# paulffm/Continuous-Time-Diffusion-Models-for-Discrete-Data

Hardware: AMD Instinct MI355X
Metric: tau-leaping sample-steps/s (higher is better)
Workload: dtype bf16; 1 GPU; MNIST tauLDR U-Net TauL step (config_tauUnet_mnist: D=784, S=256, 1000-step grid); batch_per_gpu=256, global_batch=256, D=784, S=256, parallelism=sample-sharded x1, no collective in the loop

## Files before the change

### continuous-time-diffusion-models-for-discrete-data_amd/ctdd/native.py

```python
import ctypes as C
import os

import torch

_HERE = os.path.dirname(os.path.dirname(os.path.abspath(__file__)))
_LIB = None

BRANCH_CTELBO, BRANCH_CRM = 0, 1
LOGIT_TYPES = {"direct": 0, "reverse_prob": 1, "reverse_logscale": 2}
STEP_ORDINAL, STEP_CORRECTOR, STEP_COUNT_RAW, STEP_CRM, STEP_COUNT_JUMPS, STEP_BF16, STEP_LOGITS_BF16 = 1, 2, 4, 8, 16, 32, 64


class CtddError(RuntimeError):
    pass


def lib_path():
    return os.environ.get("CTDD_LIBRARY") or os.path.join(_HERE, "libctdd.so")


_P, _I, _F, _U64, _U32, _I64 = C.c_void_p, C.c_int, C.c_float, C.c_uint64, C.c_uint32, C.c_int64
_SIGS = {
    "ctdd_abi_version": ([], _I),
    "ctdd_last_error": ([], C.c_char_p),
    "ctdd_rate_table": ([_P, _P, _P, _P, _P, _P, _I, _I, _I, _F, _P, _P, _P, _P, _P], _I),
    "ctdd_noise_categorical": ([_P, _P, _P, _P, _U64, _U64, _I, _I, _I, _P, _P], _I),
    "ctdd_xtilde_sample": ([_P, _P, _P, _P, _P, _U64, _U64, _I, _I, _I, _P, _P, _P, _P], _I),
    "ctdd_xtilde_sample_masked": ([_P, _P, _P, _P, _P, _P, _U64, _U64, _I, _I, _I, _P, _P, _P, _P], _I),
    "ctdd_logprob": ([_P, _P, _P, _P, _I, _I, _I, _I, _P, _P, _P], _I),
    "ctdd_reverse_rates": ([_I, _I, _P, _P, _P, _P, _P, _F, _I, _I, _I, _P, _P, _P], _I),
    "ctdd_tauleap_apply": ([_P, _P, _P, _I, _I, _I, _I, _P, _P, _P], _I),
    "ctdd_tauleap_draw": ([_P, _P, _P, _F, _U32, _U64, _U64, _I, _I, _I, _P, _P, _P], _I),
    "ctdd_tauleap_step": ([_I, _I, _P, _P, _P, _P, _P, _F, _F, _F, _U32, _U64, _U64, _I, _I, _I, _P, _P, _P], _I),
    "ctdd_tauleap_step_rows": ([_I, _I, _P, _P, _P, _P, _P, _F, _F, _F, _U32, _U64, _U64, _I, _I, _I, _P, _I, _P, _P, _P], _I),
    "ctdd_lbjf_step": ([_I, _I, _P, _P, _P, _P, _F, _F, _F, _U32, _P, _U64, _U64, _I, _I, _I, _P, _P, _P, _P], _I),
    "ctdd_logprob_rp_mfma": ([_P, _P, _P, _I, _I, _I, _P, _P, _P, _P], _I),
    "ctdd_logprob_rp_bwd_mfma": ([_P, _P, _P, _P, _P, _F, _I, _I, _I, _P, _P, _P, _P, _P], _I),
    "ctdd_exact_step": ([_P, _P, _P, _P, _P, _U64, _U64, _I, _I, _I, _P, _P, _P, _P], _I),
    "ctdd_midpoint_predict": ([_I, _I, _P, _P, _P, _P, _F, _F, _F, _I, _I, _I, _P, _P], _I),
    "ctdd_lbjf_from_rates": ([_P, _P, _F, _P, _U64, _U64, _I, _I, _I, _P, _P, _P, _P], _I),
    "ctdd_midpoint_from_rates": ([_P, _P, _F, _I, _I, _I, _P, _P], _I),
    "ctdd_lbjf_step_rows": ([_I, _I, _P, _P, _P, _P, _F, _F, _F, _U32, _P, _U64, _U64, _I, _I, _I, _P, _I, _P, _P, _P, _P], _I),
    "ctdd_midpoint_predict_rows": ([_I, _I, _P, _P, _P, _P, _F, _F, _F, _I, _I, _I, _P, _I, _P, _P], _I),
    "ctdd_exact_step_rows": ([_P, _P, _P, _P, _P, _U64, _U64, _I, _I, _I, _P, _I, _P, _P, _P, _P], _I),
    "ctdd_lbjf_from_rates_rows": ([_P, _P, _F, _P, _U64, _U64, _I, _I, _I, _P, _I, _P, _P, _P, _P], _I),
    "ctdd_midpoint_from_rates_rows": ([_P, _P, _F, _I, _I, _I, _P, _I, _P, _P], _I),
    "ctdd_argmax": ([_P, _I, _I, _I, _P, _P], _I),
    "ctdd_initial_samples": ([_P, _U64, _U64, _I, _I, _I, _P, _P], _I),
    "ctdd_philox_uniform": ([_U64, _U64, _I64, _I, _P, _P], _I),
    "ctdd_s256_step_table_bytes": ([], _I64),
    "ctdd_s256_prepare": ([_P, _P, _F, _I, _P, _P, _P, _P], _I),
    "ctdd_s256_prepare_crm": ([_P, _P, _I, _P, _P, _P, _P], _I),
    "ctdd_tauleap_step_s256": ([_P, _P, _P, _P, _P, _P, _F, _F, _U32, _U64, _U64, _I, _I, _P, _P, _P, _P], _I),
    "ctdd_tauleap_step_s256_rows": ([_P, _P, _P, _P, _P, _P, _F, _F, _U32, _U64, _U64, _I, _I, _P, _I, _P, _P, _P, _P], _I),
    "ctdd_crm_loss": ([_P, _P, _P, _P, _I, _I, _I, _I, _F, _F, _P, _P, _P, _P], _I),
    "ctdd_ctelbo_scratch_bytes": ([_I, _I, _I], _I64),
    "ctdd_ctelbo_loss": ([_P, _P, _P, _P, _P, _P, _I, _I, _I, _F, _F, _F, _P, _P, _P, _P], _I),
    "ctdd_ctelbo_loss_terms": ([_P, _P, _P, _P, _P, _P, _I, _I, _I, _F, _F, _F, _F, _P, _P, _P, _P], _I),
    "ctdd_ctelbo_loss_window": ([_P, _P, _P, _P, _P, _P, _I, _I, _I, _I, _I, _F, _F, _F, _F, _P, _P, _P, _P], _I),
    "ctdd_ctelbo_loss_masked": ([_P, _P, _P, _P, _P, _P, _P, _I, _I, _I, _F, _F, _F, _F, _P, _P, _P, _P], _I),
    "ctdd_score_elbo_loss": ([_P, _P, _P, _P, _P, _P, _I, _I, _I, _F, _F, _P, _P, _P, _P], _I),
    "ctdd_crm_loss_ll": ([_P, _P, _P, _I, _I, _I, _I, _F, _P, _P, _P, _P], _I),
    "ctdd_score_elbo_loss_ll": ([_P, _P, _P, _P, _P, _P, _I, _I, _I, _F, _F, _P, _P, _P, _P], _I),
    "ctdd_logprob_bwd": ([_I, _P, _P, _P, _P, _P, _F, _I, _I, _I, _P, _P, _P, _P], _I),
    "ctdd_crm_loss_masked": ([_P, _P, _P, _P, _P, _I, _I, _I, _I, _F, _F, _P, _P, _P, _P], _I),
    "ctdd_crm_loss_ll_masked": ([_P, _P, _P, _P, _I, _I, _I, _I, _F, _P, _P, _P, _P], _I),
    "ctdd_score_elbo_loss_masked": ([_P, _P, _P, _P, _P, _P, _P, _I, _I, _I, _F, _F, _P, _P, _P, _P], _I),
    "ctdd_score_elbo_loss_ll_masked": ([_P, _P, _P, _P, _P, _P, _P, _I, _I, _I, _F, _F, _P, _P, _P, _P], _I),
    "ctdd_opt_chunk_elems": ([], _I),
    "ctdd_adam_ema_step": ([_P, _P, _I, _F, _F, _F, _F, _I64, _F, _F, _P, _P], _I),
    "ctdd_grad_sumsq": ([_P, _P, _I, _P, _I, _P], _I),
    "ctdd_adam_ema_apply": ([_P, _P, _I, _F, _F, _F, _F, _I64, _F, _F, _P, _P], _I),
}
UNET_EXPORTS = ("ctdd_unet_conv", "ctdd_unet_conv_patch", "ctdd_unet_conv_res", "ctdd_unet_conv_ring", "ctdd_unet_conv_up_phases", "ctdd_unet_upsample2x", "ctdd_unet_first_conv", "ctdd_unet_gn_apply", "ctdd_unet_gn_onepass", "ctdd_unet_channel_stats",
                "ctdd_unet_time", "ctdd_unet_time_uniform", "ctdd_unet_attention", "ctdd_unet_logistic_head", "ctdd_unet_resblock_small",
                "ctdd_unet_resblock_mid", "ctdd_unet_conv_rows", "ctdd_unet_conv_rows_head")
HOLLOW_EXPORTS = ("ctdd_gemm_bf16", "ctdd_hollow_small_linear", "ctdd_hollow_embed", "ctdd_hollow_layernorm", "ctdd_hollow_add", "ctdd_hollow_put_rows", "ctdd_hollow_attention", "ctdd_hollow_attention_bf16")
UNET_TRAIN_EXPORTS = ("ctdd_unet_wgrad", "ctdd_unet_gn_bwd", "ctdd_unet_dropout", "ctdd_unet_colsum", "ctdd_unet_sum_batch", "ctdd_unet_sum_jobs", "ctdd_unet_accumulate",
                      "ctdd_unet_downsum2x", "ctdd_unet_upsample2x_f32", "ctdd_unet_cast_rows", "ctdd_unet_attention_bwd",
                      "ctdd_unet_first_conv_wgrad", "ctdd_unet_first_conv_wgrad_scratch", "ctdd_unet_pack_weights",
                      "ctdd_unet_unpack_grads")
HOLLOW_TRAIN_EXPORTS = ("ctdd_hollow_layernorm_bwd", "ctdd_hollow_attention_train", "ctdd_hollow_attention_bwd", "ctdd_hollow_attention_train_bf16", "ctdd_hollow_attention_bwd_bf16", "ctdd_hollow_act", "ctdd_hollow_relu_bf16", "ctdd_hollow_colsum", "ctdd_hollow_dropout",
                        "ctdd_hollow_embed_bwd")
BERT_EXPORTS = ("ctdd_bert_embed", "ctdd_bert_gather", "ctdd_bert_attention_short",
                "ctdd_bert_embed_bwd", "ctdd_bert_gather_bwd",
                "ctdd_bert_embed_enum_bwd", "ctdd_bert_gather_enum_bwd",
                "ctdd_bert_attention_short_train", "ctdd_bert_attention_short_bwd")
EXPORTS = tuple(_SIGS) + UNET_EXPORTS + HOLLOW_EXPORTS + UNET_TRAIN_EXPORTS + HOLLOW_TRAIN_EXPORTS + BERT_EXPORTS


def load():
    global _LIB
    if _LIB is None:
        path = lib_path()
        if not os.path.exists(path):
            raise CtddError(f"{path} not found: build it with `python __graft_entry__.py` "
                            "(hipcc --offload-arch=gfx950); there is no CPU fallback")
        lib = C.CDLL(path)
        for name, (argt, rest) in _SIGS.items():
            fn = getattr(lib, name)
            fn.argtypes, fn.restype = argt, rest
        _LIB = lib
    return _LIB


def _ptr(t, dtype=None, name="tensor"):
    if t is None:
        return None
    if not isinstance(t, torch.Tensor):
        raise CtddError(f"{name}: expected a torch tensor, got {type(t)}")
    if not t.is_cuda:
        raise CtddError(f"{name}: must live on a GPU (got {t.device}); libctdd has no CPU path")
    if dtype is not None and t.dtype != dtype:
        raise CtddError(f"{name}: expected {dtype}, got {t.dtype}")
    if not t.is_contiguous():
        raise CtddError(f"{name}: must be contiguous")
    return t.data_ptr()


def _stream():
    return torch.cuda.current_stream().cuda_stream


def _check(rc, what):
    if rc != 0:
        msg = load().ctdd_last_error().decode(errors="replace")
        raise CtddError(f"{what} failed with status {rc}: {msg}")


f32, i32 = torch.float32, torch.int32


def rate_table(eigvecs, right, eigvals, base_rate, integral, beta, S, normalise, clamp_below=1e-8,
               want_qt0=True, want_qt0T=False, want_rate=False, want_noise_probs=False):
    nT = integral.numel()
    dev = integral.device
    mk = lambda want: torch.empty((nT, S, S), dtype=f32, device=dev) if want else None
    q, qT, r, pn = mk(want_qt0), mk(want_qt0T), mk(want_rate), mk(want_noise_probs)
    rc = load().ctdd_rate_table(_ptr(eigvecs, f32, "eigvecs"), _ptr(right, f32, "right"), _ptr(eigvals, f32, "eigvals"),
                                _ptr(base_rate, f32, "base_rate"), _ptr(integral, f32, "integral"),
                                _ptr(beta, f32, "beta"), nT, S, int(bool(normalise)), float(clamp_below),
                                _ptr(q), _ptr(qT), _ptr(r), _ptr(pn), _stream())
    _check(rc, "ctdd_rate_table")
    return q, qT, r, pn


def noise_categorical(probs, x0, tidx=None, E=None, seed=0, offset=0):
    B, D = x0.shape
    S = probs.shape[-1]
    out = torch.empty((B, D), dtype=i32, device=x0.device)
    rc = load().ctdd_noise_categorical(_ptr(probs, f32, "probs"), _ptr(tidx, i32, "tidx"), _ptr(x0, i32, "x0"),
                                       _ptr(E, f32, "E"), seed, offset, B, D, S, _ptr(out), _stream())
    _check(rc, "ctdd_noise_categorical")
    return out


def xtilde_sample(rate, x_t, tidx=None, E_dim=None, E_val=None, seed=0, offset=0):
    B, D = x_t.shape
    S = rate.shape[-1]
# ... 577 lines not shown
```

### continuous-time-diffusion-models-for-discrete-data_amd/ctdd/unet_engine.py

```python
import contextlib
import ctypes as C

import torch

from . import native
from .plan_launch import bound_launch, graph_capture, ptr

_P, _I, _F = C.c_void_p, C.c_int, C.c_float
SEG_3x3, SEG_1x1, SEG_3x3_S2, SEG_3x3_UP = 0, 1, 2, 3


class _Seg(C.Structure):
    _fields_ = [("hi", _P), ("f32", _P), ("C", _I), ("kind", _I)]


class _ConvArgs(C.Structure):
    _fields_ = [("seg", _Seg * 3), ("nseg", _I), ("w_hi", _P), ("w_f32", _P), ("B", _I), ("H", _I), ("W", _I),
                ("Hin", _I), ("Win", _I), ("N", _I), ("Ktot", _I), ("bias", _P), ("tbias", _P), ("tb_stride", _I),
                ("res_f32", _P), ("res_bf16", _P), ("out_f32", _P), ("out_hi", _P), ("stats", _P), ("logits_C", _I),
                ("ksplit", _I), ("acc_buf", _P), ("act", _I), ("out_lo", _P)]


class _FirstArgs(C.Structure):
    _fields_ = [("x64", _P), ("x32", _P), ("lo", _F), ("hi", _F), ("w", _P), ("bias", _P), ("B", _I), ("Cin", _I),
                ("H", _I), ("W", _I), ("Cout", _I), ("out_f32", _P), ("out_hi", _P), ("stats", _P), ("x0_f32", _P)]


class _GnArgs(C.Structure):
    _fields_ = [("s1_f32", _P), ("s1_bf16", _P), ("st1", _P), ("C1", _I), ("s2_f32", _P), ("s2_bf16", _P), ("st2", _P),
                ("C2", _I), ("gamma", _P), ("beta", _P), ("B", _I), ("HW", _I), ("G", _I), ("eps", _F), ("swish", _I),
                ("out_hi", _P), ("out_f32", _P)]


class _ResblockArgs(C.Structure):
    _fields_ = [("s1_bf16", _P), ("s2_bf16", _P), ("C1", _I), ("C2", _I), ("gamma1", _P), ("beta1", _P), ("gamma2", _P), ("beta2", _P),
                ("G1", _I), ("G2", _I), ("eps1", _F), ("eps2", _F), ("w1", _P), ("bias1", _P), ("tbias", _P), ("tb_stride", _I),
                ("w2", _P), ("bias2", _P), ("skip", _I), ("B", _I), ("H", _I), ("W", _I), ("N", _I), ("out_bf16", _P)]


class _ConvRowsArgs(C.Structure):
    _fields_ = [("s1_bf16", _P), ("st1", _P), ("C1", _I), ("s2_bf16", _P), ("st2", _P), ("C2", _I), ("gamma", _P), ("beta", _P), ("G", _I),
                ("eps", _F), ("w", _P), ("bias", _P), ("tbias", _P), ("tb_stride", _I), ("r1_bf16", _P), ("RC1", _I), ("r2_bf16", _P),
                ("RC2", _I), ("res_bf16", _P), ("out_bf16", _P), ("out_stats", _P), ("B", _I), ("H", _I), ("W", _I), ("N", _I)]


class _TimeArgs(C.Structure):
    _fields_ = [("t", _P), ("B", _I), ("ch", _I), ("tdim", _I), ("w1", _P), ("b1", _P), ("w2", _P), ("b2", _P),
                ("hid", _P), ("act", _P)]


class _AttnArgs(C.Structure):
    _fields_ = [("qkv", _P), ("B", _I), ("T", _I), ("C", _I), ("heads", _I), ("out_hi", _P), ("out_f32", _P)]


class _LogisticArgs(C.Structure):
    _fields_ = [("net", _P), ("x0", _P), ("B", _I), ("C", _I), ("HW", _I), ("S", _I), ("fix", _I), ("out", _P), ("fast", _I), ("out_bf16", _P)]


_sigs_done = False


def _lib():
    global _sigs_done
    lib = native.load()
    if not _sigs_done:
        for name, argt in (("ctdd_unet_conv", [_P, _I, _I, _I, _P]), ("ctdd_unet_conv_patch", [_P, _I, _I, _I, _P]), ("ctdd_unet_conv_res", [_P, _I, _P]), ("ctdd_unet_conv_ring", [_P, _I, _P]),
                           ("ctdd_unet_conv_up_phases", [_P, _I, _P]), ("ctdd_unet_upsample2x", [_P, _I, _I, _I, _I, _P, _P]), ("ctdd_unet_first_conv", [_P, _P]),
                           ("ctdd_unet_gn_apply", [_P, _P]), ("ctdd_unet_gn_onepass", [_P, _I, _I, _P]), ("ctdd_unet_channel_stats", [_P, _I, _I, _I, _P, _P]),
                           ("ctdd_unet_time", [_P, _P, _P, _I, _P, _P]), ("ctdd_unet_time_uniform", [_P, _P, _P, _I, _P, _P]),
                           ("ctdd_unet_attention", [_P, _P]), ("ctdd_unet_resblock_small", [_P, _I, _P]),
                           ("ctdd_unet_resblock_mid", [_P, _I, _P]), ("ctdd_unet_conv_rows", [_P, _I, _P]),
                           ("ctdd_unet_conv_rows_head", [_P, _I, _P]),
                           ("ctdd_unet_logistic_head", [_P, _P])):
            fn = getattr(lib, name)
            fn.argtypes, fn.restype = argt, _I
        _sigs_done = True
    return lib


def _unwrap(net):
    return net.module if hasattr(net, "module") and net.__class__.__name__ == "DistributedDataParallel" else net


def supports(model):
    net = _unwrap(getattr(model, "net", None))
    return (net is not None and net.__class__.__name__ == "UNet" and not model.padding
            and model.cfg.model.model_output in ("logits", "logistic_pars"))


def training_supported(model):
    if getattr(model.cfg.model, "engine_train", "hip") != "hip" or not supports(model):
        return False
    net = _unwrap(model.net)
    return net.channel % 16 == 0 and all((net.channel * int(m_)) % 16 == 0 for m_ in model.cfg.model.ch_mult)



def resblock_small_covers(H, W, cs, cout, G1, G2):
    Ct = sum(cs)
    if H * W > 64 or W > 8 or cout != 192 or len(cs) > 2 or any(c % 64 for c in cs) or Ct > 384 or Ct % G1 or cout % G2:
        return False
    if H * W > 16 and (H - 1) * (W + 2) + W > 80:
        return False
    rs_a, rs_2, prows = Ct * 2 + 32, cout * 2 + 32, (H + 2) * (W + 2)
    return H * W * rs_a + prows * max(rs_a, rs_2) + 256 * 80 + 2 * 384 * 8 + 2 * 384 * 4 <= 160 * 1024


def pack_resblock_weights(w2d):
    N, K = w2d.shape
    assert N == 192 and K % 64 == 0
    return w2d.reshape(4, 3, 16, K // 64, 2, 4, 8).permute(0, 3, 1, 4, 5, 2, 6).contiguous().reshape(N, K)


def resblock_mid_covers(H, W, cs, cout, G1, G2):
    Ct = sum(cs)
    if (H < 1 or W < 1 or H > 14 or W > 14 or cout != 192 or not 1 <= len(cs) <= 2
            or any(c <= 0 or c % 32 or c > 192 for c in cs) or G1 <= 0 or G2 <= 0 or Ct % G1 or cout % G2):
        return False
    return ((H + 2) * 16 + 2) * (cout * 2 + 32) + 256 * 80 + 2 * 384 * 8 + 2 * 384 * 4 <= 160 * 1024


def pack_row_tile_weights(w, cs, rcs, streams):
    N, Ct, Rt = w.shape[0], sum(cs), sum(rcs)
    assert N == 48 * streams and w.shape[1] == 9 * Ct + Rt and all(c % 32 == 0 for c in [*cs, *rcs])
    w3, parts, c0 = w[:, :9 * Ct].reshape(N, 9, Ct), [], 0
    for c in cs:
        v = w3[:, :, c0:c0 + c].reshape(streams, 3, 16, 3, 3, c // 32, 4, 8)
        parts.append(v.permute(0, 5, 4, 3, 1, 6, 2, 7).reshape(streams, -1))
        c0 += c
    c0 = 9 * Ct
    for c in rcs:
        v = w[:, c0:c0 + c].reshape(streams, 3, 16, c // 32, 4, 8)
        parts.append(v.permute(0, 3, 1, 4, 2, 5).reshape(streams, -1))
        c0 += c
    return torch.cat(parts, 1).contiguous().reshape(N, w.shape[1])


def pack_resblock_mid_weights(w1, w2, cs):
    N = w1.shape[0]
    return pack_row_tile_weights(w1, cs, [], 4), pack_row_tile_weights(w2, [N], cs if w2.shape[1] > 9 * N else [], 4)


def pack_conv_rows_weights(w, cs, rcs):
    return pack_row_tile_weights(w, cs, rcs, 2)


CONV_ROWS_MIN_WGS = 96


def conv_rows_covers(H, W, cs, rcs, cout, G, residual=False):
    return bool(H >= 1 and 1 <= W <= 28 and cout == 96 and 1 <= len(cs) <= 2 and len(rcs) <= 2 and all(c > 0 and c % 32 == 0 for c in [*cs, *rcs])
                and sum(cs) <= 384 and sum(rcs) <= 384 and G > 0 and sum(cs) % G == 0 and not (rcs and residual))


def pack_conv_rows_head_weights(w, C1):
    N, passes = w.shape[0], -(-w.shape[0] // 96)
    wp = torch.zeros((96 * passes, w.shape[1]), dtype=w.dtype, device=w.device)
    wp[:N] = w
    return pack_row_tile_weights(wp, [C1], [], 2 * passes)


HEAD_ROWS_MIN_WGS = 192


def conv_rows_head_covers(H, W, C1, N, G):
    return bool(H >= 1 and 1 <= W <= 28 and C1 in (32, 64, 96) and G > 0 and C1 % G == 0 and 32 <= N <= 576 and N % 32 == 0)


def fold_upsample_weights(w):
    N, Cn = w.shape[:2]
    assert tuple(w.shape[2:]) == (3, 3)
    sel = torch.tensor([[[1, 0, 0], [0, 1, 1]], [[1, 1, 0], [0, 0, 1]]], dtype=w.dtype, device=w.device)
    return torch.einsum("pia,qjb,ncab->pqnijc", sel, sel, w).reshape(4, N, 4 * Cn).contiguous()


def upsample_phases_covers(B, Hs, Ws, Cn, N):
    return bool(Cn >= 16 and Cn % 16 == 0 and (N % 96 == 0 or N % 64 == 0) and N > 0 and 1 <= Ws <= 33 and Hs * Ws >= 32
                and 4 * Cn * 64 < 2 ** 31 and 4 * B * Hs * Ws < 2 ** 31)


def _onepass_slab(B, HW, Cn, G, max_threads=1024):
    if Cn % 8 or G <= 0 or Cn % G:
        return 0
    cg = Cn // G
    L = cg
    while L % 8:
        L += cg
    best = 0
    for sc in range(L, Cn + 1, L):
        if Cn % sc:
            continue
        noct = sc // 8
        if noct > max_threads:
            continue
# ... 251 lines not shown
        self.launch(self.lib.ctdd_unet_conv_rows_head, C.byref(a), 0, label=f"{src.H}x{src.W} K={9 * C1} N={N} gn+conv rows head C={[C1]}",
                    flops=2 * B * src.H * src.W * N * 9 * C1)

    def conv2_operands(self, rb, a2, srcs):
        tc = self.tc
        segs, wsrc, bias_params = [(a2, rb.conv2.weight.shape[0], SEG_3x3)], [(rb.conv2.weight, 0)], [rb.conv2.bias]
        bias = rb.conv2.bias.detach().float()
        if rb.skip is not None:
            c_ = 0
            for s_ in srcs:
                segs.append((s_, s_.C, SEG_1x1))
                wsrc.append((rb.skip.weight, c_))
                c_ += s_.C
            bias_params.append(rb.skip.bias)
            bias = tc.summed_bias(bias_params) if tc is not None else bias + rb.skip.bias.detach().float()
        return segs, wsrc, bias_params, bias.contiguous()

    def resblock_fused(self, rb, srcs, mid=False):
        eng, lib, B = self.eng, self.lib, self.B
        Hc, Wc = srcs[0].H, srcs[0].W
        cs = [s.C for s in srcs]
        Ct, cout = sum(cs), rb.conv1.weight.shape[0]
        y = _Tensor(self, Hc, Wc, cout)
        a = _ResblockArgs()
        a.s1_bf16, a.C1 = ptr(srcs[0].hi), cs[0]
        if len(srcs) == 2:
            a.s2_bf16, a.C2 = ptr(srcs[1].hi), cs[1]
        par = [p_.detach().float().contiguous() for p_ in (rb.norm1.weight, rb.norm1.bias, rb.norm2.weight, rb.norm2.bias, rb.conv1.bias)]
        a.gamma1, a.beta1, a.gamma2, a.beta2, a.bias1 = (ptr(p_) for p_ in par)
        a.G1, a.G2, a.eps1, a.eps2 = rb.norm1.num_groups, rb.norm2.num_groups, rb.norm1.eps, rb.norm2.eps
        a.tbias, a.tb_stride = self.tproj.data_ptr() + 4 * self.toff[id(rb)], self.tb_stride
        w1 = eng._w2d([(rb.conv1.weight, 0)], [(None, Ct, SEG_3x3)])
        segs, wsrc, _, bias2 = self.conv2_operands(rb, None, srcs)
        w2 = eng._w2d(wsrc, segs)
        w1, w2 = pack_resblock_mid_weights(w1, w2, cs) if mid else (pack_resblock_weights(w1), pack_resblock_weights(w2))
        (w1, _), (w2, _) = eng._pack(w1), eng._pack(w2)
        a.w1, a.w2, a.bias2, a.skip = ptr(w1), ptr(w2), ptr(bias2), int(rb.skip is not None)
        a.B, a.H, a.W, a.N, a.out_bf16 = B, Hc, Wc, cout, ptr(y.hi)
        self.keep.extend(par + [w1, w2, bias2, a])
        K1, K2 = w1.shape[1], w2.shape[1]
        self.launch(lib.ctdd_unet_resblock_mid if mid else lib.ctdd_unet_resblock_small, C.byref(a), 0,
                    label=f"{Hc}x{Wc} resblock C={cs} N={cout} K={K1}+{K2}", flops=2 * B * Hc * Wc * cout * (9 * Ct + 9 * cout + (Ct if rb.skip is not None else 0)))
        return y

    def resblock(self, rb, srcs):
        eng, tc = self.eng, self.tc
        Hc, Wc = srcs[0].H, srcs[0].W
        cs = [s.C for s in srcs]
        cout = rb.conv1.weight.shape[0]
        if self.onepass_gn and eng._fuses_resblock(rb, Hc, Wc, cs, tc is not None) and all(s_.stats is None for s_ in srcs):
            return self.resblock_fused(rb, srcs)
        if self.onepass_gn and eng._fuses_resblock_mid(rb, Hc, Wc, cs, tc is not None) and all(s_.stats is None for s_ in srcs):
            return self.resblock_fused(rb, srcs, mid=True)
        tbias = (self.tproj.data_ptr() + 4 * self.toff[id(rb)], self.tb_stride)
        h = _Tensor(self, Hc, Wc, cout)
        b1 = rb.conv1.bias.detach().float().contiguous()
        if eng._runs_conv_rows(self.B, Hc, Wc, cs, [], cout, rb.norm1.num_groups, False, tc is not None) and all(s_.stats is not None for s_ in srcs):
            self.conv_rows(srcs, rb.norm1, [(None, sum(cs), SEG_3x3)], [(rb.conv1.weight, 0)], b1, h, tb=tbias)
        else:
            a1 = self.gn_apply(srcs, rb.norm1, True, rb.norm1.eps, Hc * Wc)
            self.conv([(a1, a1.C, SEG_3x3)], [(rb.conv1.weight, 0)], b1, cout, Hc, Wc, Hc, Wc, h, tb=tbias, bias_params=[rb.conv1.bias])
        rcs, res = (cs, None) if rb.skip is not None else ([], srcs[0])
        if eng._runs_conv_rows(self.B, Hc, Wc, [cout], rcs, cout, rb.norm2.num_groups, rb.skip is None, tc is not None) and h.stats is not None:
            y = _Tensor(self, Hc, Wc, cout)
            segs, wsrc, _, bias2 = self.conv2_operands(rb, None, srcs)
            self.conv_rows([h], rb.norm2, segs, wsrc, bias2, y, res=res, raws=srcs if rb.skip is not None else ())
            return y
        drop = float(rb.dropout.p) if (tc is not None and tc.dropout) else 0.0
        a2 = self.gn_apply([h], rb.norm2, True, rb.norm2.eps, Hc * Wc, drop_p=drop)
        y = _Tensor(self, Hc, Wc, cout)
        segs, wsrc, bias_params, bias2 = self.conv2_operands(rb, a2, srcs)
        self.conv(segs, wsrc, bias2, cout, Hc, Wc, Hc, Wc, y, res=res, bias_params=bias_params)
        return y

    def block(self, layer, srcs):
        cur = self.resblock(layer.resblocks, srcs)
        return cur if layer.attention is None else self.attention(layer.attention, cur)

    def attention(self, att, x):
        tc, lib, B = self.tc, self.lib, self.B
        T = x.H * x.W
        an = self.gn_apply([x], att.norm, False, att.norm.eps, T)
        Cx = x.C
        qkv = torch.empty((B * T, 3 * Cx), dtype=torch.float32, device=self.dev)
        self.keep.append(qkv)
        self.conv([(an, Cx, SEG_1x1)], [(att.qkv.weight, 0)],
                  att.qkv.bias.detach().float().contiguous(), 3 * Cx, x.H, x.W, x.H, x.W, None, out_f32_tensor=qkv,
                  bias_params=[att.qkv.bias])
        ao = _Tensor(self, x.H, x.W, Cx, stats=False)
        aa = _AttnArgs()
        aa.qkv, aa.B, aa.T, aa.C, aa.heads, aa.out_hi, aa.out_f32 = ptr(qkv), B, T, Cx, att.num_heads, ptr(ao.hi), ptr(ao.f32)
        self.keep.extend([aa, ao])
        self.launch(lib.ctdd_unet_attention, C.byref(aa))
        if tc is not None:
            tc.record_attention(att, qkv, ao, B, T, Cx)
        y = _Tensor(self, x.H, x.W, Cx)
        self.conv([(ao, Cx, SEG_1x1)], [(att.proj_out.weight, 0)],
                  att.proj_out.bias.detach().float().contiguous(), Cx, x.H, x.W, x.H, x.W, y, res=x, bias_params=[att.proj_out.bias])
        return y

    def time(self, uniform_t):
        tc, B, st, lib, dev, ch = self.tc, self.B, self.st, self.lib, self.dev, self.net.channel
        resblocks, pw, pb, tw = self.eng._time_weights()
        tdim, Ntot = ch * 4, pw.shape[1]
        st.tact = torch.empty((B, tdim), dtype=torch.float32, device=dev)
        time_row = uniform_t == "row" and tc is None
        uniform_t = bool(uniform_t) and tc is None
        st.time_row = time_row
        self.tproj = st.tproj = torch.empty((1 if uniform_t else B, Ntot), dtype=torch.float32, device=dev)
        self.tb_stride = 0 if uniform_t else Ntot
        ta = _TimeArgs()
        st.thid = torch.empty((B, tdim), dtype=torch.float32, device=dev)
        ta.t, ta.B, ta.ch, ta.tdim = ptr(st.t_in), B, ch, tdim
        ta.w1, ta.b1, ta.w2, ta.b2, ta.hid, ta.act = ptr(tw[0]), ptr(tw[1]), ptr(tw[2]), ptr(tw[3]), ptr(st.thid), ptr(st.tact)
        self.keep.extend(tw + [pw, pb, ta])
        if tc is None and not time_row:
            self.launch(lib.ctdd_unet_time_uniform if uniform_t else lib.ctdd_unet_time, C.byref(ta), ptr(pw), ptr(pb), Ntot, ptr(st.tproj))
        elif tc is None:
            st.tproj.zero_()
        else:
            tc.tproj, tc.resblocks = st.tproj, resblocks
        self.toff, o = {}, 0
        for rb in resblocks:
            self.toff[id(rb)] = o
            o += rb.time[1].weight.shape[0]

    def first_conv(self, c0):
        st, B, net, ch, (Cin, H0, W0) = self.st, self.B, self.net, self.net.channel, self.shape
        cur = _Tensor(self, H0, W0, ch)
        fa = _FirstArgs()
        if st.x_in.dtype == torch.int64:
            fa.x64 = ptr(st.x_in)
        else:
            fa.x32 = ptr(st.x_in)
        fa.lo, fa.hi = float(net.x_min_max[0]), float(net.x_min_max[1])
        w0, b0 = c0.weight.detach().float().contiguous(), c0.bias.detach().float().contiguous()
        fa.w, fa.bias, fa.B, fa.Cin, fa.H, fa.W, fa.Cout = ptr(w0), ptr(b0), B, Cin, H0, W0, ch
        fa.out_f32, fa.out_hi = ptr(cur.f32), ptr(cur.hi)
        if self.m.model_output == "logistic_pars":
            st.x0 = torch.empty((B, Cin, H0, W0), dtype=torch.float32, device=self.dev)
            fa.x0_f32 = ptr(st.x0)
        if cur.stats is not None:
            self.stats_views.append((fa, cur.stats, "stats"))
        self.keep.extend([w0, b0, fa])
        self.launch(self.lib.ctdd_unet_first_conv, C.byref(fa))
        if self.tc is not None:
            self.tc.record_first(c0, fa, cur)
        return cur

    def downsample(self, cv, cur):
        Ho, Wo = (cur.H + 1 - 3) // 2 + 1, (cur.W + 1 - 3) // 2 + 1
        y = _Tensor(self, Ho, Wo, cur.C)
        self.conv([(cur, cur.C, SEG_3x3_S2)], [(cv.weight, 0)],
                  cv.bias.detach().float().contiguous(), cur.C, Ho, Wo, cur.H, cur.W, y, bias_params=[cv.bias])
        return y

    def upsample_in_phases(self, cur):
        eng, m, B, Cn = self.eng, self.m, self.B, cur.C
        if self.tc is not None or eng.precise or not int(getattr(m, "upsample_phases", 1)):
            return False
        Ho, Wo = cur.H * 2, cur.W * 2
        ring = self.pick_kernel(True, B * Ho * Wo, Cn, Ho, Wo) == "ring" and Wo <= 33 and Cn % 32 == 0
        if not ring or (getattr(m, "conv_ksplit", 1) > 1 and Cn // 16 >= 2) or getattr(m, "ring_small_tiles", 0):
            return False
        return upsample_phases_covers(B, cur.H, cur.W, Cn, Cn)

    def upsample_phases(self, cv, cur, y):
        eng, B, Cn = self.eng, self.B, cur.C
        a = _ConvArgs()
        a.nseg = 1
        a.seg[0].hi, a.seg[0].C, a.seg[0].kind = ptr(cur.hi), Cn, SEG_3x3_UP
        whi, _ = eng._pack(fold_upsample_weights(cv.weight.detach().float()).reshape(4 * Cn, 4 * Cn))
        bias = cv.bias.detach().float().contiguous()
        a.w_hi, a.bias = ptr(whi), ptr(bias)
        a.B, a.H, a.W, a.Hin, a.Win, a.N, a.Ktot = B, y.H, y.W, cur.H, cur.W, Cn, 4 * Cn
        a.out_hi = ptr(y.hi)
        if y.stats is not None and not y.stats_by_gn:
            self.stats_views.append((a, y.stats, "stats"))
        self.keep.extend([whi, bias, a])
        self.launch(self.lib.ctdd_unet_conv_up_phases, C.byref(a), 0, label=f"{y.H}x{y.W} K=4x{4 * Cn} N={Cn} up-phases of {cur.H}x{cur.W}",
                    flops=2 * B * y.H * y.W * Cn * 4 * Cn)
# ... 64 lines not shown
            feats.append(cur)
        for layer in net.mid:
            cur = self.block(layer, [cur])
        for layer in net.up:
            cur = self.block(layer, [cur, feats.pop()]) if hasattr(layer, "resblocks") else self.upsample(layer[1], cur)
        self.head(cur, logits_out, logits_bf16)
        if self.tc is not None:
            self.tc.finish(self)
        st.stats = torch.zeros((max(self.stats_off, 1),), dtype=torch.float64, device=dev)
        base = st.stats.data_ptr()
        for a_, off, field in self.stats_views:
            setattr(a_, field, base + 8 * off)
        nz = sum(n for _, n in self.zero_views)
        st.zpool = torch.zeros((max(nz, 1),), dtype=torch.float32, device=dev)
        zo = 0
        for a_, n in self.zero_views:
            a_.acc_buf = st.zpool.data_ptr() + 4 * zo
            zo += n
        st.plan, st.keep, st.graph = self.plan, self.keep, None
        return st


class UNetEngine:
    def __init__(self, model, precision=None):
        self.model = model
        self.net = _unwrap(model.net)
        self.cfg = model.cfg
        self.dev = next(self.net.parameters()).device
        if self.dev.type != "cuda":
            raise native.CtddError("UNetEngine needs the model on a GPU")
        self.precision = precision or getattr(self.cfg.model, "engine_precision", "bf16")
        if self.precision not in ("bf16", "fp32"):
            raise ValueError(f"unknown engine precision {self.precision}")
        self.precise = self.precision == "fp32"
        self._plans = {}
        self._wver = None
        self._time_w = None

    def _weights_version(self):
        return sum(p._version for p in self.net.parameters()) + 7919 * getattr(self.model, "_weights_version", 0)

    def _pack(self, w2d):
        w = w2d.detach().float().contiguous()
        return (None, w) if self.precise else (w.to(torch.bfloat16).contiguous(), None)

    @staticmethod
    def _w2d(wsrc, segs):
        parts = []
        for (w, c_off), (_, cs, kind) in zip(wsrc, segs):
            w = w.detach().float()
            N = w.shape[0]
            if kind == SEG_1x1:
                parts.append(w.reshape(N, -1)[:, c_off:c_off + cs])
            else:
                parts.append(w[:, c_off:c_off + cs].permute(0, 2, 3, 1).reshape(N, 9 * cs))
        return torch.cat(parts, dim=1).contiguous()


    def _time_weights(self):
        ver = self._weights_version()
        if self._time_w is None or self._time_w[0] != ver:
            net = self.net
            resblocks = [mod.resblocks for mod in list(net.down) + list(net.mid) + list(net.up) if hasattr(mod, "resblocks")]
            pw = torch.cat([rb.time[1].weight.detach().float() for rb in resblocks], 0).t().contiguous()
            pb = torch.cat([rb.time[1].bias.detach().float() for rb in resblocks], 0).contiguous()
            tw = [net.time[1].weight.t(), net.time[1].bias, net.time[3].weight.t(), net.time[3].bias]
            tw = [w.detach().float().contiguous() for w in tw]
            self._time_w = (ver, resblocks, pw, pb, tw)
        return self._time_w[1:]

    def _onepass_max_hw(self):
        return int(getattr(self.cfg.model, "gn_onepass_max_hw", 256))

    def _fuses_resblock(self, rb, Hc, Wc, cs, training):
        return bool(not training and not self.precise and int(getattr(self.cfg.model, "resblock_fused", 1))
                    and Hc * Wc <= self._onepass_max_hw()
                    and resblock_small_covers(Hc, Wc, cs, rb.conv1.weight.shape[0], rb.norm1.num_groups, rb.norm2.num_groups))

    def _fuses_resblock_mid(self, rb, Hc, Wc, cs, training):
        return bool(not training and not self.precise and int(getattr(self.cfg.model, "resblock_fused_mid", 1))
                    and Hc * Wc <= self._onepass_max_hw()
                    and not resblock_small_covers(Hc, Wc, cs, rb.conv1.weight.shape[0], rb.norm1.num_groups, rb.norm2.num_groups)
                    and resblock_mid_covers(Hc, Wc, cs, rb.conv1.weight.shape[0], rb.norm1.num_groups, rb.norm2.num_groups))

    def _runs_conv_rows(self, B, Hc, Wc, cs, rcs, cout, G, residual, training):
        m = self.cfg.model
        return bool(not training and not self.precise and int(getattr(m, "conv_rows", 1))
                    and conv_rows_covers(Hc, Wc, cs, rcs, cout, G, residual)
                    and B * -(-Hc // 14) >= int(getattr(m, "conv_rows_min_wgs", CONV_ROWS_MIN_WGS)))

    def _runs_head_rows(self, B, Hc, Wc, C1, N, G, training):
        m = self.cfg.model
        return bool(not training and not self.precise and int(getattr(m, "conv_rows", 1)) and int(getattr(m, "head_rows", 1))
                    and conv_rows_head_covers(Hc, Wc, C1, N, G)
                    and B * -(-Hc // 14) >= int(getattr(m, "head_rows_min_wgs", HEAD_ROWS_MIN_WGS)))

    def _onepass_gn_covers(self, B, training):
        net, (_, H, W) = self.net, self.cfg.data.shape
        max_hw, threads = self._onepass_max_hw(), int(getattr(self.cfg.model, "gn_threads", 512))
        norms, c = [], net.channel
        for layer in [*list(net.down)[1:], *net.mid, *net.up]:
            if hasattr(layer, "downsample"):
                H, W = (H + 1 - 3) // 2 + 1, (W + 1 - 3) // 2 + 1
            elif not hasattr(layer, "resblocks"):
                H, W = 2 * H, 2 * W
            else:
                rb, c1 = layer.resblocks, layer.resblocks.norm1.num_channels
                cs = [c] if c1 == c else [c, c1 - c]
                if not (self._fuses_resblock(rb, H, W, cs, training) or self._fuses_resblock_mid(rb, H, W, cs, training)):
                    norms += [(H * W, rb.norm1), (H * W, rb.norm2)]
                c = rb.norm2.num_channels
                if layer.attention is not None:
                    norms.append((H * W, layer.attention.norm))
        norms.append((H * W, net.out[0]))
        return all(hw > max_hw or _onepass_slab(B, hw, n.num_channels, n.num_groups, threads) > 0 for hw, n in norms)

    def _build(self, B, x_dtype, logits_out=None, tc=None, logits_bf16=False, uniform_t=False):
        m = self.cfg.model
        onepass_gn = bool((not self.precise) and int(getattr(m, "gn_onepass", 1)) and (tc is None or int(getattr(m, "gn_onepass_train", 1)))
                          and self._onepass_gn_covers(B, tc is not None))
        return _PlanBuilder(self, B, tc, onepass_gn).build(x_dtype, logits_out, logits_bf16, uniform_t)

    def _run_plan(self, st):
        st.stats.zero_()
        st.zpool.zero_()
        for step in st.plan:
            step()

    def _prepare(self, B, x_dtype, x, times, logits_out=None, logits_bf16=False, uniform_t=False, time_row=None):
        st = self._build(B, x_dtype, logits_out, logits_bf16=logits_bf16, uniform_t=uniform_t)
        st.x_in.copy_(x.reshape(st.x_in.shape))
        self._set_time(st, times, time_row)
        self._run_plan(st)
        torch.cuda.synchronize()
        (st.graph,) = self._capture([lambda: self._run_plan(st)], "", "the plan runs as eager launches")
        return st

    def _capture(self, runs, what, then):
        if getattr(self.cfg.model, "engine_graph", True):
            try:
                graphs = []
                for run in runs:
                    graphs.append(torch.cuda.CUDAGraph())
                    with graph_capture(graphs[-1]):
                        run()
                return graphs
            except native.CtddError:
                raise
            except RuntimeError as e:
                import warnings
                warnings.warn(f"[ctdd] UNetEngine: HIP-graph capture{what} failed ({e}); {then}", RuntimeWarning)
                torch.cuda.synchronize()
        return [None] * len(runs)

    @staticmethod
    def _set_time(st, times, time_row):
        if st.time_row:
            if time_row is None or time_row.numel() != st.tproj.numel():
                raise native.CtddError("UNetEngine: this plan takes a precomputed time-projection row (time_table()[i])")
            st.tproj.copy_(time_row.reshape(st.tproj.shape))
        else:
            st.t_in.copy_(times.float())

    @staticmethod
    def _replay(st, x, times, time_row=None):
        st.x_in.copy_(x.reshape(st.x_in.shape))
# ... 168 lines not shown
```

### include/ctdd_unet.h

```cpp
#ifndef CTDD_UNET_H
#define CTDD_UNET_H
#include <stdint.h>
#ifdef __cplusplus
extern "C" {
#endif

#define CTDD_SEG_3x3 0
#define CTDD_SEG_1x1 1
#define CTDD_SEG_3x3_S2 2
#define CTDD_SEG_3x3_UP 3
#define CTDD_SEG_3x3_S2T 4

typedef struct { const void* hi; const float* f32; int C, kind; } ctdd_conv_seg;
typedef struct {
  ctdd_conv_seg seg[3]; int nseg;
  const void* w_hi; const float* w_f32;
  int B, H, W, Hin, Win, N, Ktot;
  const float* bias; const float* tbias; int tb_stride;
  const float* res_f32; const void* res_bf16;
  float* out_f32; void* out_hi; double* stats; int logits_C;
  int ksplit; float* acc_buf;
  int act;
  void* out_lo;
} ctdd_conv_args;
int ctdd_unet_conv(const void* conv_args, int bk, int bnt, int f32, void* stream);
int ctdd_unet_conv_patch(const void* conv_args, int bk, int bnt, int wm, void* stream);
int ctdd_unet_conv_res(const void* conv_args, int bnt, void* stream);
int ctdd_unet_conv_ring(const void* conv_args, int bnt, void* stream);
int ctdd_unet_conv_up_phases(const void* conv_args, int f32, void* stream);
int ctdd_unet_upsample2x(const void* x_bf16,int B, int H, int W, int C, void* out_bf16, void* stream);

typedef struct {
  const int64_t* x64; const int32_t* x32; float lo, hi; const float* w; const float* bias;
  int B, Cin, H, W, Cout; float* out_f32; void* out_hi; double* stats; float* x0_f32;
} ctdd_first_conv_args;
int ctdd_unet_first_conv(const void* first_conv_args, void* stream);

typedef struct {
  const float* s1_f32; const void* s1_bf16; const double* st1; int C1;
  const float* s2_f32; const void* s2_bf16; const double* st2; int C2;
  const float* gamma; const float* beta; int B, HW, G; float eps; int swish; void* out_hi; float* out_f32;
} ctdd_gn_args;
int ctdd_unet_gn_apply(const void* gn_args, void* stream);
int ctdd_unet_gn_onepass(const void* gn_args, int slab_channels, int max_threads, void* stream);
int ctdd_unet_channel_stats(const float* x, int B, int HW, int C, double* stats, void* stream);

typedef struct {
  const void* s1_bf16; const void* s2_bf16; int C1, C2;
  const float* gamma1; const float* beta1; const float* gamma2; const float* beta2; int G1, G2; float eps1, eps2;
  const void* w1; const float* bias1; const float* tbias; int tb_stride;
  const void* w2; const float* bias2;
  int skip;
  int B, H, W, N; void* out_bf16;
} ctdd_resblock_args;
int ctdd_unet_resblock_small(const void* resblock_args, int f32, void* stream);
int ctdd_unet_resblock_mid(const void* resblock_args, int f32, void* stream);

typedef struct {
  const void* s1_bf16; const double* st1; int C1;
  const void* s2_bf16; const double* st2; int C2;
  const float* gamma; const float* beta; int G; float eps;
  const void* w; const float* bias; const float* tbias; int tb_stride;
  const void* r1_bf16; int RC1; const void* r2_bf16; int RC2;
  const void* res_bf16;
  void* out_bf16; double* out_stats;
  int B, H, W, N;
} ctdd_conv_rows_args;
int ctdd_unet_conv_rows(const void* conv_rows_args, int f32, void* stream);
int ctdd_unet_conv_rows_head(const void* conv_rows_args, int f32, void* stream);

typedef struct {
  const float* t; int B, ch, tdim;
  const float* w1; const float* b1; const float* w2; const float* b2;
  float* hid; float* act;
} ctdd_time_args;
int ctdd_unet_time(const void* time_args, const float* proj_w, const float* proj_b, int Ntot, float* proj_out, void* stream);
int ctdd_unet_time_uniform(const void* time_args, const float* proj_w, const float* proj_b, int Ntot, float* proj_out, void* stream);

typedef struct { const float* qkv; int B, T, C, heads; void* out_hi; float* out_f32; } ctdd_attn_args;
int ctdd_unet_attention(const void* attn_args, void* stream);

typedef struct { const float* net; const float* x0; int B, C, HW, S, fix; float* out;
                 int fast;
                 void* out_bf16;    } ctdd_logistic_args;
int ctdd_unet_logistic_head(const void* logistic_args, void* stream);

#ifdef __cplusplus
}
#endif
#endif
```

Before: 131,100 sample-steps/s.

## Fuse U-Net attention block (QKV, softmax attention, projection, residual) into one kernel

Adds a single-workgroup-per-sample HIP kernel that does the QKV 1x1 conv with bf16 MFMA, per-head softmax attention in LDS with fp32 MFMA, the output projection, and the residual add. It covers attention layers with T<=64 tokens, C=192 and 8 heads. This replaces three launches and the fp32 qkv and attention-output round trips through global memory. The trade-offs are one workgroup per sample using up to a full CU's LDS, which limits occupancy, and a kernel tied to a fixed shape.

After: 134,400 sample-steps/s, median of 6. 2.5% higher.

```diff
diff --git a/continuous-time-diffusion-models-for-discrete-data_amd/csrc/unet_attn_kernels.hip b/continuous-time-diffusion-models-for-discrete-data_amd/csrc/unet_attn_kernels.hip
--- /dev/null
+++ b/continuous-time-diffusion-models-for-discrete-data_amd/csrc/unet_attn_kernels.hip
@@ -0,0 +1,247 @@
+#include "row_tile.hpp"
+#include "../../include/ctdd_unet.h"
+
+namespace ctdd {
+namespace {
+
+constexpr int AB_THREADS = 256, AB_C = 192, AB_HEADS = 8, AB_CH = AB_C / AB_HEADS, AB_TP = 64;
+constexpr int AB_RS = AB_C * 2 + 32;
+constexpr int AB_HROW = (3 * AB_CH + 4) * 4;
+constexpr int AB_HREG = AB_TP * AB_HROW;
+constexpr int AB_LDS = AB_HEADS * AB_HREG;
+constexpr int AB_KS = AB_C / 32;
+constexpr int AB_NQT = 3 * AB_C / 64;
+static_assert(AB_TP * AB_RS <= AB_LDS && AB_CH % 4 == 0 && AB_CH % 8 == 0 && AB_CH > 16 && AB_CH <= 32 && AB_NQT * 16 == 2 * 3 * AB_CH, "tile geometry");
+
+__global__ __launch_bounds__(AB_THREADS, 1) void k_attn_block(const ctdd_attn_block_args a) {
+  extern __shared__ __attribute__((aligned(16))) unsigned char sm[];
+  const int t = threadIdx.x, b = blockIdx.x, T = a.T;
+  const int lane = t & 63, wv = t >> 6, lj = lane & 15, lq = lane >> 4;
+  const unsigned short* wq = (const unsigned short*)a.w_qkv + (size_t)wv * (AB_KS * AB_NQT * 512) + lane * 8;
+  const unsigned short* wp = (const unsigned short*)a.w_proj + (size_t)wv * (AB_KS * 3 * 512) + lane * 8;
+
+  constexpr int NV = AB_C / 8, MAXV = AB_TP * NV / AB_THREADS;
+  const unsigned short* an = (const unsigned short*)a.an_bf16 + (size_t)b * T * AB_C;
+  u32x4 u[MAXV];
+#pragma unroll
+  for (int k = 0; k < MAXV; ++k) {
+    const int v = t + k * AB_THREADS, p = v / NV, c8 = v - p * NV, pc = p < T ? p : T - 1;
+    u[k] = *(const u32x4*)(an + (size_t)pc * AB_C + c8 * 8);
+  }
+  asm volatile("" ::: "memory");
+  f32x4 acc[AB_NQT][4];
+#pragma unroll
+  for (int tt = 0; tt < AB_NQT; ++tt) {
+    const float4 bv = *(const float4*)(a.b_qkv + wv * (AB_NQT * 16) + 16 * tt + 4 * lq);
+#pragma unroll
+    for (int pt = 0; pt < 4; ++pt) acc[tt][pt] = (f32x4){bv.x, bv.y, bv.z, bv.w};
+  }
+  u32x4 wr[AB_KS][AB_NQT];
+#pragma unroll
+  for (int ks = 0; ks < AB_KS; ++ks)
+#pragma unroll
+    for (int tt = 0; tt < AB_NQT; ++tt) wr[ks][tt] = *(const u32x4*)(wq + (ks * AB_NQT + tt) * 512);
+#pragma unroll
+  for (int k = 0; k < MAXV; ++k) {
+    const int v = t + k * AB_THREADS, p = v / NV, c8 = v - p * NV;
+    *(u32x4*)(sm + p * AB_RS + c8 * 16) = p < T ? u[k] : (u32x4){0u, 0u, 0u, 0u};
+  }
+  __syncthreads();
+
+#pragma unroll
+  for (int ks = 0; ks < AB_KS; ++ks) {
+    bf16x8 xf[4];
+#pragma unroll
+    for (int pt = 0; pt < 4; ++pt) xf[pt] = *(const bf16x8*)(sm + (16 * pt + lj) * AB_RS + ks * 64 + lq * 16);
+#pragma unroll
+    for (int tt = 0; tt < AB_NQT; ++tt)
+#pragma unroll
+      for (int pt = 0; pt < 4; ++pt)
+        acc[tt][pt] = __builtin_amdgcn_mfma_f32_16x16x32_bf16(__builtin_bit_cast(bf16x8, wr[ks][tt]), xf[pt], acc[tt][pt], 0, 0, 0);
+  }
+  __syncthreads();
+
+  u32x4 wpj[AB_KS][3];
+#pragma unroll
+  for (int ks = 0; ks < AB_KS; ++ks)
+#pragma unroll
+    for (int tt = 0; tt < 3; ++tt) wpj[ks][tt] = *(const u32x4*)(wp + (ks * 3 + tt) * 512);
+  const unsigned short* xs = (const unsigned short*)a.x_bf16 + (size_t)b * T * AB_C;
+  uint2 xr[3][4];
+  f32x4 pa[3][4];
+#pragma unroll
+  for (int tt = 0; tt < 3; ++tt) {
+    const float4 bv = *(const float4*)(a.b_proj + wv * 48 + tt * 16 + lq * 4);
+#pragma unroll
+    for (int pt = 0; pt < 4; ++pt) {
+      const int p = 16 * pt + lj, pc = p < T ? p : T - 1;
+      xr[tt][pt] = *(const uint2*)(xs + (size_t)pc * AB_C + wv * 48 + tt * 16 + lq * 4);
+      pa[tt][pt] = (f32x4){bv.x, bv.y, bv.z, bv.w};
+    }
+  }
+
+  {
+    const float sc = 1.0f / sqrtf(sqrtf((float)AB_CH));
+#pragma unroll
+    for (int tt = 0; tt < AB_NQT; ++tt) {
+      const int cw = 16 * tt + 4 * lq, hh = cw >= 3 * AB_CH ? 1 : 0, cc = cw - hh * 3 * AB_CH;
+      const float mul = cc < 2 * AB_CH ? sc : 1.0f;
+      unsigned char* dst = sm + (2 * wv + hh) * AB_HREG + cc * 4;
+#pragma unroll
+      for (int pt = 0; pt < 4; ++pt) {
+        const f32x4 v = acc[tt][pt];
+        *(float4*)(dst + (16 * pt + lj) * AB_HROW) = make_float4(v[0] * mul, v[1] * mul, v[2] * mul, v[3] * mul);
+      }
+    }
+  }
+  __syncthreads();
+
+#pragma unroll 1
+  for (int hh = 0; hh < 2; ++hh) {
+    unsigned char* R = sm + (2 * wv + hh) * AB_HREG;
+    float kf[AB_CH / 4][4], qf[AB_CH / 4][4];
+#pragma unroll
+    for (int st = 0; st < AB_CH / 4; ++st)
+#pragma unroll
+      for (int i = 0; i < 4; ++i) {
+        qf[st][i] = *(const float*)(R + (16 * i + lj) * AB_HROW + (4 * st + lq) * 4);
+        kf[st][i] = *(const float*)(R + (16 * i + lj) * AB_HROW + (AB_CH + 4 * st + lq) * 4);
+      }
+    float vf[4][4][2];
+#pragma unroll
+    for (int si = 0; si < 4; ++si)
+#pragma unroll
+      for (int r = 0; r < 4; ++r)
+#pragma unroll
+        for (int ci = 0; ci < 2; ++ci) {
+          const int c = 16 * ci + lj < AB_CH ? 16 * ci + lj : AB_CH - 1;
+          vf[si][r][ci] = *(const float*)(R + (16 * si + 4 * lq + r) * AB_HROW + (2 * AB_CH + c) * 4);
+        }
+    f32x4 S[4][4];
+#pragma unroll
+    for (int si = 0; si < 4; ++si) {
+      f32x4 s0;
+#pragma unroll
+      for (int r = 0; r < 4; ++r) s0[r] = 16 * si + 4 * lq + r < T ? 0.0f : -INFINITY;
+#pragma unroll
+      for (int ti = 0; ti < 4; ++ti) S[si][ti] = s0;
+    }
+#pragma unroll
+    for (int st = 0; st < AB_CH / 4; ++st)
+#pragma unroll
+      for (int si = 0; si < 4; ++si)
+#pragma unroll
+        for (int ti = 0; ti < 4; ++ti) S[si][ti] = __builtin_amdgcn_mfma_f32_16x16x4f32(kf[st][si], qf[st][ti], S[si][ti], 0, 0, 0);
+
+    float rz[4];
+#pragma unroll
+    for (int ti = 0; ti < 4; ++ti) {
+      float m = -INFINITY;
+#pragma unroll
+      for (int si = 0; si < 4; ++si)
+#pragma unroll
+        for (int r = 0; r < 4; ++r) m = fmaxf(m, S[si][ti][r]);
+      m = fmaxf(m, __shfl_xor(m, 16, WAVE));
+      m = fmaxf(m, __shfl_xor(m, 32, WAVE));
+      float z = 0.0f;
+#pragma unroll
+      for (int si = 0; si < 4; ++si)
+#pragma unroll
+        for (int r = 0; r < 4; ++r) {
+          const float e = __builtin_amdgcn_exp2f((S[si][ti][r] - m) * 1.4426950408889634f);
+          S[si][ti][r] = e;
+          z += e;
+        }
+      z += __shfl_xor(z, 16, WAVE);
+      z += __shfl_xor(z, 32, WAVE);
+      rz[ti] = 1.0f / z;
+    }
+
+    f32x4 O[2][4];
+#pragma unroll
+    for (int ci = 0; ci < 2; ++ci)
+#pragma unroll
+      for (int ti = 0; ti < 4; ++ti) O[ci][ti] = (f32x4){0.0f, 0.0f, 0.0f, 0.0f};
+#pragma unroll
+    for (int si = 0; si < 4; ++si)
+#pragma unroll
+      for (int r = 0; r < 4; ++r) {
+        if (16 * si + r >= T) continue;
+#pragma unroll
+        for (int ci = 0; ci < 2; ++ci)
+#pragma unroll
+          for (int ti = 0; ti < 4; ++ti) O[ci][ti] = __builtin_amdgcn_mfma_f32_16x16x4f32(vf[si][r][ci], S[si][ti][r], O[ci][ti], 0, 0, 0);
+      }
+#pragma unroll
+    for (int ci = 0; ci < 2; ++ci) {
+      const int c0 = 16 * ci + 4 * lq;
+      if (c0 < AB_CH) {
+#pragma unroll
+        for (int ti = 0; ti < 4; ++ti) {
+          const f32x4 o = O[ci][ti];
+          const float r_ = rz[ti];
+          *(uint2*)(R + (16 * ti + lj) * AB_HROW + c0 * 2) = make_uint2(rt_pack2(o[0] * r_, o[1] * r_), rt_pack2(o[2] * r_, o[3] * r_));
+        }
+      }
+    }
+  }
+  __syncthreads();
+
+#pragma unroll
+  for (int ks = 0; ks < AB_KS; ++ks) {
+    constexpr int PER = AB_CH / 8;
+    const int cb = 4 * ks + lq, hd = cb / PER, off = (cb - hd * PER) * 16;
+    bf16x8 xf[4];
+#pragma unroll
+    for (int pt = 0; pt < 4; ++pt) xf[pt] = *(const bf16x8*)(sm + hd * AB_HREG + (16 * pt + lj) * AB_HROW + off);
+#pragma unroll
+    for (int tt = 0; tt < 3; ++tt)
+#pragma unroll
+      for (int pt = 0; pt < 4; ++pt)
+        pa[tt][pt] = __builtin_amdgcn_mfma_f32_16x16x32_bf16(__builtin_bit_cast(bf16x8, wpj[ks][tt]), xf[pt], pa[tt][pt], 0, 0, 0);
+  }
+  unsigned short* out = (unsigned short*)a.out_bf16 + (size_t)b * T * AB_C;
+#pragma unroll
+  for (int tt = 0; tt < 3; ++tt) {
+    const int n = wv * 48 + tt * 16 + lq * 4;
+#pragma unroll
+    for (int pt = 0; pt < 4; ++pt) {
+      const int p = 16 * pt + lj;
+      if (p < T) {
+        const f32x4 v = pa[tt][pt];
+        const uint2 r = xr[tt][pt];
+        const float o0 = v[0] + __uint_as_float(r.x << 16), o1 = v[1] + __uint_as_float(r.x & 0xFFFF0000u);
+        const float o2 = v[2] + __uint_as_float(r.y << 16), o3 = v[3] + __uint_as_float(r.y & 0xFFFF0000u);
+        *(uint2*)(out + (size_t)p * AB_C + n) = make_uint2(rt_pack2(o0, o1), rt_pack2(o2, o3));
+      }
+    }
+  }
+}
+
+}
+}
+
+using namespace ctdd;
+
+extern "C" int ctdd_unet_attention_block(const void* args_, int f32, void* stream) {
+  CTDD_REQUIRE(args_, CTDD_EINVAL, "ctdd_unet_attention_block: null arguments");
+  const ctdd_attn_block_args& a = *(const ctdd_attn_block_args*)args_;
+  CTDD_REQUIRE(f32 == 0, CTDD_ERANGE, "ctdd_unet_attention_block: bf16 inference only (the fp32 mode keeps the three launches)");
+  CTDD_REQUIRE(a.B > 0 && a.T > 0 && a.C > 0 && a.heads > 0 && a.C % a.heads == 0, CTDD_EINVAL,
+               "ctdd_unet_attention_block: bad shape (B=%d, T=%d, C=%d, heads=%d)", a.B, a.T, a.C, a.heads);
+  CTDD_REQUIRE((a.C / a.heads) % 4 == 0, CTDD_ERANGE, "ctdd_unet_attention_block: head width %d is not a multiple of 4", a.C / a.heads);
+  CTDD_REQUIRE(a.C == AB_C && a.heads == AB_HEADS, CTDD_ERANGE, "ctdd_unet_attention_block: C=%d in %d heads is off the tile (C = 192, 8 heads)", a.C,
+               a.heads);
+  CTDD_REQUIRE(a.T <= AB_TP, CTDD_ERANGE, "ctdd_unet_attention_block: T=%d tokens do not fit the workgroup tile (T <= 64: an LDS image within 160 KiB)",
+               a.T);
+  CTDD_REQUIRE(a.an_bf16 && a.x_bf16 && a.w_qkv && a.b_qkv && a.w_proj && a.b_proj && a.out_bf16, CTDD_EINVAL,
+               "ctdd_unet_attention_block: null pointer");
+  const uintptr_t al = (uintptr_t)a.an_bf16 | (uintptr_t)a.x_bf16 | (uintptr_t)a.w_qkv | (uintptr_t)a.b_qkv | (uintptr_t)a.w_proj |
+                       (uintptr_t)a.b_proj | (uintptr_t)a.out_bf16;
+  CTDD_REQUIRE((al & 15) == 0, CTDD_EINVAL, "ctdd_unet_attention_block: tensors must be 16-byte aligned");
+  static_assert(AB_LDS <= 160 * 1024, "LDS image over the CU's 160 KiB");
+  static bool attr_done[16] = {};
+  ensure_lds_ceiling((const void*)k_attn_block, attr_done);
+  hipLaunchKernelGGL(k_attn_block, dim3(a.B), dim3(AB_THREADS), (size_t)AB_LDS, (hipStream_t)stream, a);
+  return finish_launch("k_attn_block");
+}
diff --git a/continuous-time-diffusion-models-for-discrete-data_amd/ctdd/native.py b/continuous-time-diffusion-models-for-discrete-data_amd/ctdd/native.py
--- a/continuous-time-diffusion-models-for-discrete-data_amd/ctdd/native.py
+++ b/continuous-time-diffusion-models-for-discrete-data_amd/ctdd/native.py
@@ -74,7 +74,7 @@
 }
 UNET_EXPORTS = ("ctdd_unet_conv", "ctdd_unet_conv_patch", "ctdd_unet_conv_res", "ctdd_unet_conv_ring", "ctdd_unet_conv_up_phases", "ctdd_unet_upsample2x", "ctdd_unet_first_conv", "ctdd_unet_gn_apply", "ctdd_unet_gn_onepass", "ctdd_unet_channel_stats",
                 "ctdd_unet_time", "ctdd_unet_time_uniform", "ctdd_unet_attention", "ctdd_unet_logistic_head", "ctdd_unet_resblock_small",
-                "ctdd_unet_resblock_mid", "ctdd_unet_conv_rows", "ctdd_unet_conv_rows_head")
+                "ctdd_unet_resblock_mid", "ctdd_unet_conv_rows", "ctdd_unet_conv_rows_head", "ctdd_unet_attention_block")
 HOLLOW_EXPORTS = ("ctdd_gemm_bf16", "ctdd_hollow_small_linear", "ctdd_hollow_embed", "ctdd_hollow_layernorm", "ctdd_hollow_add", "ctdd_hollow_put_rows", "ctdd_hollow_attention", "ctdd_hollow_attention_bf16")
 UNET_TRAIN_EXPORTS = ("ctdd_unet_wgrad", "ctdd_unet_gn_bwd", "ctdd_unet_dropout", "ctdd_unet_colsum", "ctdd_unet_sum_batch", "ctdd_unet_sum_jobs", "ctdd_unet_accumulate",
                       "ctdd_unet_downsum2x", "ctdd_unet_upsample2x_f32", "ctdd_unet_cast_rows", "ctdd_unet_attention_bwd",
diff --git a/continuous-time-diffusion-models-for-discrete-data_amd/ctdd/unet_engine.py b/continuous-time-diffusion-models-for-discrete-data_amd/ctdd/unet_engine.py
--- a/continuous-time-diffusion-models-for-discrete-data_amd/ctdd/unet_engine.py
+++ b/continuous-time-diffusion-models-for-discrete-data_amd/ctdd/unet_engine.py
@@ -51,6 +51,11 @@
 
 class _AttnArgs(C.Structure):
     _fields_ = [("qkv", _P), ("B", _I), ("T", _I), ("C", _I), ("heads", _I), ("out_hi", _P), ("out_f32", _P)]
+
+
+class _AttnBlockArgs(C.Structure):
+    _fields_ = [("an_bf16", _P), ("x_bf16", _P), ("w_qkv", _P), ("b_qkv", _P), ("w_proj", _P), ("b_proj", _P), ("B", _I), ("T", _I),
+                ("C", _I), ("heads", _I), ("out_bf16", _P)]
 
 
 class _LogisticArgs(C.Structure):
@@ -68,7 +73,8 @@
                            ("ctdd_unet_conv_up_phases", [_P, _I, _P]), ("ctdd_unet_upsample2x", [_P, _I, _I, _I, _I, _P, _P]), ("ctdd_unet_first_conv", [_P, _P]),
                            ("ctdd_unet_gn_apply", [_P, _P]), ("ctdd_unet_gn_onepass", [_P, _I, _I, _P]), ("ctdd_unet_channel_stats", [_P, _I, _I, _I, _P, _P]),
                            ("ctdd_unet_time", [_P, _P, _P, _I, _P, _P]), ("ctdd_unet_time_uniform", [_P, _P, _P, _I, _P, _P]),
-                           ("ctdd_unet_attention", [_P, _P]), ("ctdd_unet_resblock_small", [_P, _I, _P]),
+                           ("ctdd_unet_attention", [_P, _P]), ("ctdd_unet_attention_block", [_P, _I, _P]),
+                           ("ctdd_unet_resblock_small", [_P, _I, _P]),
                            ("ctdd_unet_resblock_mid", [_P, _I, _P]), ("ctdd_unet_conv_rows", [_P, _I, _P]),
                            ("ctdd_unet_conv_rows_head", [_P, _I, _P]),
                            ("ctdd_unet_logistic_head", [_P, _P])):
@@ -110,6 +116,16 @@
     N, K = w2d.shape
     assert N == 192 and K % 64 == 0
     return w2d.reshape(4, 3, 16, K // 64, 2, 4, 8).permute(0, 3, 1, 4, 5, 2, 6).contiguous().reshape(N, K)
+
+
+def attention_block_covers(T, Cn, heads):
+    return bool(1 <= T <= 64 and Cn == 192 and heads == 8)
+
+
+def pack_attention_weights(w2d):
+    N, K = w2d.shape
+    assert N % 64 == 0 and K % 32 == 0
+    return w2d.reshape(4, N // 64, 16, K // 32, 4, 8).permute(0, 3, 1, 4, 2, 5).contiguous().reshape(N, K)
 
 
 def resblock_mid_covers(H, W, cs, cout, G1, G2):
@@ -527,6 +543,8 @@
         T = x.H * x.W
         an = self.gn_apply([x], att.norm, False, att.norm.eps, T)
         Cx = x.C
+        if self.onepass_gn and T <= self.no_stats_hw and self.eng._fuses_attention(att, T, Cx, tc is not None):
+            return self.attention_fused(att, x, an)
         qkv = torch.empty((B * T, 3 * Cx), dtype=torch.float32, device=self.dev)
         self.keep.append(qkv)
         self.conv([(an, Cx, SEG_1x1)], [(att.qkv.weight, 0)],
@@ -542,6 +560,19 @@
         y = _Tensor(self, x.H, x.W, Cx)
         self.conv([(ao, Cx, SEG_1x1)], [(att.proj_out.weight, 0)],
                   att.proj_out.bias.detach().float().contiguous(), Cx, x.H, x.W, x.H, x.W, y, res=x, bias_params=[att.proj_out.bias])
+        return y
+
+    def attention_fused(self, att, x, an):
+        eng, B, T, Cx = self.eng, self.B, x.H * x.W, x.C
+        y = _Tensor(self, x.H, x.W, Cx)
+        (wq, _), (wp, _) = (eng._pack(pack_attention_weights(w.detach().float().reshape(w.shape[0], Cx))) for w in (att.qkv.weight, att.proj_out.weight))
+        bq, bp = att.qkv.bias.detach().float().contiguous(), att.proj_out.bias.detach().float().contiguous()
+        a = _AttnBlockArgs()
+        a.an_bf16, a.x_bf16, a.w_qkv, a.b_qkv, a.w_proj, a.b_proj = ptr(an.hi), ptr(x.hi), ptr(wq), ptr(bq), ptr(wp), ptr(bp)
+        a.B, a.T, a.C, a.heads, a.out_bf16 = B, T, Cx, att.num_heads, ptr(y.hi)
+        self.keep.extend([wq, bq, wp, bp, a])
+        self.launch(self.lib.ctdd_unet_attention_block, C.byref(a), 0, label=f"{x.H}x{x.W} attention block C={Cx} heads={att.num_heads}",
+                    flops=2 * B * T * Cx * (3 * Cx + Cx))
         return y
 
     def time(self, uniform_t):
@@ -772,6 +803,10 @@
                     and Hc * Wc <= self._onepass_max_hw()
                     and not resblock_small_covers(Hc, Wc, cs, rb.conv1.weight.shape[0], rb.norm1.num_groups, rb.norm2.num_groups)
                     and resblock_mid_covers(Hc, Wc, cs, rb.conv1.weight.shape[0], rb.norm1.num_groups, rb.norm2.num_groups))
+
+    def _fuses_attention(self, att, T, Cn, training):
+        return bool(not training and not self.precise and int(getattr(self.cfg.model, "attention_fused", 1))
+                    and attention_block_covers(T, Cn, att.num_heads))
 
     def _runs_conv_rows(self, B, Hc, Wc, cs, rcs, cout, G, residual, training):
         m = self.cfg.model
diff --git a/include/ctdd_unet.h b/include/ctdd_unet.h
--- a/include/ctdd_unet.h
+++ b/include/ctdd_unet.h
@@ -80,6 +80,14 @@
 typedef struct { const float* qkv; int B, T, C, heads; void* out_hi; float* out_f32; } ctdd_attn_args;
 int ctdd_unet_attention(const void* attn_args, void* stream);
 
+typedef struct {
+  const void* an_bf16; const void* x_bf16;
+  const void* w_qkv; const float* b_qkv;
+  const void* w_proj; const float* b_proj;
+  int B, T, C, heads; void* out_bf16;
+} ctdd_attn_block_args;
+int ctdd_unet_attention_block(const void* attn_block_args, int f32, void* stream);
+
 typedef struct { const float* net; const float* x0; int B, C, HW, S, fix; float* out;
                  int fast;
                  void* out_bf16;    } ctdd_logistic_args;
```
